# THUDM/GCC

Hardware: NVIDIA B200
Metric: subgraphs/sec (MoCo pretrain step) (higher is better)
Workload: dtype f32

## Files before the change

gcc_b200/csrc/gin_bwd.cu:

```cuda
#include "gin_common.cuh"
#include "tc_gemm.cuh"
#ifndef GCCB_EMU
#include <cuda_bf16.h>
#endif

namespace gccb {

#define GCCB_WG_CHUNKS 148

struct BwdLayout {
  size_t dh, g1[2], dz2[2], da, red, dS, dpool, part, total;
  size_t dz16, tA, tB, coef1, splitk;
  int DW;
  int cap_pad, splits;
};

inline BwdLayout make_bwd_layout(const GinDims& d, int B, int node_cap) {
  BwdLayout b;
  size_t off = 0;
  auto take = [&](size_t bytes) { size_t o = off; off += (bytes + 255) & ~(size_t)255; return o; };
  b.DW = d.H > GCCB_DINP ? d.H : GCCB_DINP;
  b.dh = take((size_t)node_cap * b.DW * 4);
  for (int i = 0; i < 2; ++i) {
    b.g1[i] = take((size_t)node_cap * d.H * 4);
    b.dz2[i] = take((size_t)node_cap * d.H * 4);
  }
  b.da = take((size_t)node_cap * b.DW * 4);
  b.red = take((size_t)(d.L - 1) * 3 * 2 * d.H * 8);
  b.dS = take((size_t)d.L * B * d.H * 4);
  b.dpool = take((size_t)d.L * B * b.DW * 4);
  b.part = take((size_t)GCCB_WG_CHUNKS * ((size_t)d.H * b.DW + d.H) * 4);
  b.dz16 = b.tA = b.tB = b.coef1 = b.splitk = 0;
  b.cap_pad = (node_cap + 63) & ~63;
  b.splits = 0;
#ifndef GCCB_EMU
  if (d.tc) {
    b.dz16 = take((size_t)node_cap * d.H * 2);
    b.tA = take((size_t)d.H * b.cap_pad * 2);
    b.tB = take((size_t)b.DW * b.cap_pad * 2);
    b.coef1 = take((size_t)(d.L - 1) * 2 * d.H * 4);
    const int tiles = (d.H / 128) * 1;
    b.splits = 148 / tiles;
    if (b.splits > b.cap_pad / 64) b.splits = b.cap_pad / 64;
// ... 90 lines not shown
  const int idx = blockIdx.x * blockDim.x + threadIdx.x;
  if (idx < H * inf) {
    const int o = idx / inf, k = idx - o * inf;
    float s = 0.f;
    for (int g = 0; g < B; ++g)
      s = fmaf(dS[((size_t)l * B + g) * H + o], pooled[((size_t)l * B + g) * PW + k], s);
    grads[lay.wp[l] + idx] += s;
  } else if (idx < H * inf + H) {
    const int o = idx - H * inf;
    float s = 0.f;
    for (int g = 0; g < B; ++g) s += dS[((size_t)l * B + g) * H + o];
    grads[lay.bp[l] + o] += s;
  }
}

template <int W>
__global__ void __launch_bounds__(256)
gin_bwd_dh_kernel(const int32_t* __restrict__ node_off_v, int B, const int32_t* __restrict__ indptr,
                  const int32_t* __restrict__ indices, const int32_t* __restrict__ graph_id,
                  const float* __restrict__ dpool_j, int DW, const float* __restrict__ da, int has_da,
                  float* __restrict__ dh) {
  __shared__ float scratch[8 * W];
  __shared__ int hub_rows[GCCB_HUB_QUEUE];
  __shared__ int n_hub;
  const int N = node_off_v[B];
  const int tid = threadIdx.x, lane = tid & 31, warp = tid >> 5;
  constexpr int V4 = W / 4, PERV = (V4 + 31) / 32;
  if (tid == 0) n_hub = 0;
  __syncthreads();
  for (int r = blockIdx.x * 8 + warp; r < N; r += gridDim.x * 8) {
    const int beg = indptr[r], end = indptr[r + 1];
    if (has_da && end - beg > GCCB_HUB_DEG) {
      int slot = GCCB_HUB_QUEUE;
      if (lane == 0) slot = atomicAdd(&n_hub, 1);
      slot = __shfl_sync(0xffffffffu, slot, 0);
      if (slot < GCCB_HUB_QUEUE) {
        if (lane == 0) hub_rows[slot] = r;
        continue;
      }
    }
    const int g = graph_id[r];
    float4 acc[PERV];
// ... 1 lines not shown
    for (int j = 0; j < PERV; ++j) {
      const int v = lane + 32 * j;
      acc[j] = make_float4(0.f, 0.f, 0.f, 0.f);
      if (v < V4) {
        acc[j] = *reinterpret_cast<const float4*>(dpool_j + (size_t)g * DW + 4 * v);
        if (has_da) {
          const float4 x = *reinterpret_cast<const float4*>(da + (size_t)r * W + 4 * v);
          acc[j].x += x.x; acc[j].y += x.y; acc[j].z += x.z; acc[j].w += x.w;
        }
      }
    }
    if (has_da) gather_range4<W>(da, indices, beg, end, lane, acc);
#pragma unroll
    for (int j = 0; j < PERV; ++j) {
      const int v = lane + 32 * j;
      if (v < V4) *reinterpret_cast<float4*>(dh + (size_t)r * W + 4 * v) = acc[j];
    }
  }
  __syncthreads();
  const int nh = min(n_hub, GCCB_HUB_QUEUE);
  for (int hi = 0; hi < nh; ++hi) {
    const int rh = hub_rows[hi];
    const float s = gather_hub<W>(da, indices, indptr[rh], indptr[rh + 1], scratch);
    if (tid < W) dh[(size_t)rh * W + tid] = dpool_j[(size_t)graph_id[rh] * DW + tid] + da[(size_t)rh * W + tid] + s;
  }
}

struct BnC { const float *mean, *invstd, *sc, *sh; };
__device__ __forceinline__ BnC bnc(const float* p, int H) { BnC b; b.mean = p; b.invstd = p + H; b.sc = p + 2 * H; b.sh = p + 3 * H; return b; }

__device__ __forceinline__ void chain_g4(float z2v, float dhv, const BnC& A, const BnC& Bc, int c,
                                         float* ya, float* yhat, float* g4) {
  float yap = fmaf(z2v, A.sc[c], A.sh[c]);
  float y = fmaxf(yap, 0.f);
  float hb = fmaf(y, Bc.sc[c], Bc.sh[c]);
  *ya = yap;
  *yhat = (y - Bc.mean[c]) * Bc.invstd[c];
  *g4 = hb > 0.f ? dhv : 0.f;
}

template <int H>
__global__ void __launch_bounds__(256)
gin_bwd_reduce_kernel(int mode, const int32_t* __restrict__ node_off_v, int B,
                      const float* __restrict__ z2, const float* __restrict__ dh,
                      const double* __restrict__ sums_a, const float* __restrict__ ga,
                      const float* __restrict__ bea, const double* __restrict__ sums_b,
                      const float* __restrict__ gb, const float* __restrict__ beb, float bn_eps,
                      const double* __restrict__ redB_in, double* __restrict__ red_out) {
  __shared__ float coef_a[4 * H];
  __shared__ float coef_b[4 * H];
  __shared__ float red[2 * 1024];
  const int N = node_off_v[B];
  const int tid = threadIdx.x;
  bn_prepare(sums_a, N, H, ga, bea, bn_eps, coef_a, coef_a + H, coef_a + 2 * H, coef_a + 3 * H, nullptr, false, false, 0.f);
  bn_prepare(sums_b, N, H, gb, beb, bn_eps, coef_b, coef_b + H, coef_b + 2 * H, coef_b + 3 * H, nullptr, false, false, 0.f);
  __syncthreads();
  const BnC A = bnc(coef_a, H), Bc = bnc(coef_b, H);
  constexpr int TPR = H / 4, RP = 256 / TPR;
  const int c4 = (tid % TPR) * 4, rsub = tid / TPR;
  const float invN = N > 0 ? 1.0f / (float)N : 0.f;
  float m_g4[4] = {0.f, 0.f, 0.f, 0.f}, m_g4y[4] = {0.f, 0.f, 0.f, 0.f};
  if (mode == 1) {
#pragma unroll
    for (int k = 0; k < 4; ++k) { m_g4[k] = (float)(redB_in[c4 + k] * invN); m_g4y[k] = (float)(redB_in[H + c4 + k] * invN); }
  }
  float s[4] = {0.f, 0.f, 0.f, 0.f}, q[4] = {0.f, 0.f, 0.f, 0.f};
  const int stride = gridDim.x * RP;
  for (int r = blockIdx.x * RP + rsub; r < N; r += 2 * stride) {
    float4 zv[2], dv[2];
#pragma unroll
    for (int u = 0; u < 2; ++u) {
      const int rr = r + u * stride;
      const bool ok = rr < N;
      zv[u] = ok ? *reinterpret_cast<const float4*>(z2 + (size_t)rr * H + c4) : make_float4(0.f, 0.f, 0.f, 0.f);
      dv[u] = ok ? *reinterpret_cast<const float4*>(dh + (size_t)rr * H + c4) : make_float4(0.f, 0.f, 0.f, 0.f);
    }
#pragma unroll
    for (int u = 0; u < 2; ++u) {
      if (r + u * stride < N) {
        const float zz[4] = {zv[u].x, zv[u].y, zv[u].z, zv[u].w}, dd[4] = {dv[u].x, dv[u].y, dv[u].z, dv[u].w};
#pragma unroll
        for (int k = 0; k < 4; ++k) {
          const int c = c4 + k;
          float ya, yhat, g4;
          chain_g4(zz[k], dd[k], A, Bc, c, &ya, &yhat, &g4);
          if (mode == 0) {
            s[k] += g4;
            q[k] = fmaf(g4, yhat, q[k]);
          } else {
            const float dy = Bc.sc[c] * (g4 - m_g4[k] - yhat * m_g4y[k]);
            const float g3 = ya > 0.f ? dy : 0.f;
            const float z2hat = (zz[k] - A.mean[c]) * A.invstd[c];
            s[k] += g3;
            q[k] = fmaf(g3, z2hat, q[k]);
          }
        }
      }
    }
  }
#pragma unroll
  for (int k = 0; k < 4; ++k) {
    red[(0 * RP + rsub) * H + c4 + k] = s[k];
    red[(RP + rsub) * H + c4 + k] = q[k];
  }
  __syncthreads();
  for (int idx = tid; idx < 2 * H; idx += 256) {
    int which = idx / H, cc = idx - which * H;
    float t = 0.f;
    for (int j = 0; j < RP; ++j) t += red[(which * RP + j) * H + cc];
    atomicAdd(&red_out[which * H + cc], (double)t);
// ... 151 lines not shown
#pragma unroll
    for (int i = 0; i < 4; ++i) {
      const int r = row0 + ty * 4 + i;
      if (r < N) {
#pragma unroll
        for (int c = 0; c < TC::CPT; ++c) da_out[(size_t)r * KIN + TC::col(tx, c)] = acc[i][c];
      }
    }
  }
}

__global__ void __launch_bounds__(256)
gin_wgrad_kernel(const int32_t* __restrict__ node_off_v, int B, int H, int KQ,
                 const float* __restrict__ P, const float* __restrict__ Q,
                 const double* __restrict__ q_sums, const float* __restrict__ q_gamma,
                 const float* __restrict__ q_beta, float bn_eps, float* __restrict__ part) {
  __shared__ float Ps[GCCB_TILE_ROWS][65];
  __shared__ float Qs[GCCB_TILE_ROWS][65];
  __shared__ float qsc[64], qsh[64];
  const int N = node_off_v[B];
  const int tid = threadIdx.x, tx = tid & 15, ty = tid >> 4;
  const int kblocks = (KQ + 63) / 64;
  const int ob = blockIdx.y / kblocks, kb = blockIdx.y - ob * kblocks;
  const int o0 = ob * 64, k0 = kb * 64;
  const bool xform = q_sums != nullptr;
  if (xform) {
    for (int c = tid; c < 64; c += 256) {
      int k = k0 + c;
      float sc = 0.f, sh = 0.f;
      if (k < KQ) {
        double n = N > 0 ? (double)N : 1.0;
// ... 48 lines not shown
    }
    if (kb == 0 && tid < 64)
      for (int rr = 0; rr < GCCB_TILE_ROWS; ++rr) bacc += Ps[rr][tid];
  }
  float* mypart = part + (size_t)blockIdx.x * ((size_t)H * KQ + H);
#pragma unroll
  for (int i = 0; i < 4; ++i) {
    int o = o0 + ty * 4 + i;
#pragma unroll
    for (int j = 0; j < 4; ++j) {
      int k = k0 + tx * 4 + j;
      if (o < H && k < KQ) mypart[(size_t)o * KQ + k] = acc[i][j];
    }
  }
  if (kb == 0 && tid < 64 && o0 + tid < H) mypart[(size_t)H * KQ + o0 + tid] = bacc;
}

__global__ void __launch_bounds__(256)
gin_wgrad_reduce_kernel(int H, int KQ, int in_features, const float* __restrict__ part,
                        float* __restrict__ gw, float* __restrict__ gb) {
  const int idx = blockIdx.x * blockDim.x + threadIdx.x;
  const size_t stride = (size_t)H * KQ + H;
  if (idx < H * KQ) {
    const int o = idx / KQ, k = idx - o * KQ;
    if (k < in_features) {
      float s0 = 0.f, s1 = 0.f, s2 = 0.f, s3 = 0.f;
      for (int ch = 0; ch < GCCB_WG_CHUNKS; ch += 4) {
        s0 += part[(ch + 0) * stride + idx]; s1 += part[(ch + 1) * stride + idx];
        s2 += part[(ch + 2) * stride + idx]; s3 += part[(ch + 3) * stride + idx];
      }
      gw[(size_t)o * in_features + k] += (s0 + s1) + (s2 + s3);
    }
  } else if (idx < H * KQ + H) {
    float s = 0.f;
    for (int ch = 0; ch < GCCB_WG_CHUNKS; ++ch) s += part[ch * stride + idx];
    gb[idx - H * KQ] += s;
  }
}

__global__ void gin_bn_grads_kernel(int H, const double* __restrict__ red, float* __restrict__ gw,
                                    float* __restrict__ gb) {
  int c = blockIdx.x * blockDim.x + threadIdx.x;
  if (c < H) { gb[c] += (float)red[c]; gw[c] += (float)red[H + c]; }
}

__global__ void __launch_bounds__(256)
gin_bwd_emb_kernel(GinDims d, const int32_t* __restrict__ node_off_v, int B,
                   const int32_t* __restrict__ sub_deg, const float* __restrict__ dx0,
                   float* __restrict__ gemb) {
  GCCB_DYN_SMEM(float, hist);
  const int N = node_off_v[B];
  const int cells = (d.maxdeg + 1) * d.D;
  for (int i = threadIdx.x; i < cells; i += blockDim.x) hist[i] = 0.f;
  __syncthreads();
  const int total = N * d.D;
  for (int idx = blockIdx.x * blockDim.x + threadIdx.x; idx < total; idx += gridDim.x * blockDim.x) {
    int r = idx / d.D, c = idx - r * d.D;
    int dg = sub_deg[r];
// ... 31 lines not shown
  const int32_t* node_off_v = a.batch->node_off + (size_t)a.view * (B + 1);
  const int32_t* indptr = a.batch->indptr + (size_t)a.view * (cap + 1);
  const int32_t* indices = a.batch->indices + (size_t)a.view * a.batch->edge_cap;
  const int32_t* sub_deg = a.batch->sub_deg + (size_t)a.view * cap;
  const int32_t* graph_id = a.batch->graph_id + (size_t)a.view * cap;
  const double* stats = (const double*)(a.acts + a.al.stats);
  float* dh = (float*)(a.ws + a.bl.dh);
  float* da = (float*)(a.ws + a.bl.da);
  double* red = (double*)(a.ws + a.bl.red);
  float* dS = (float*)(a.ws + a.bl.dS);
  float* dpool = (float*)(a.ws + a.bl.dpool);
  float* part = (float*)(a.ws + a.bl.part);
  const float* P = a.params;
  float* G = a.grads;
  const int DW = a.bl.DW;
  const int tiles = (cap + GCCB_TILE_ROWS - 1) / GCCB_TILE_ROWS;
  const int grid = tiles < 592 ? tiles : 592;
  const uint32_t keep = (uint32_t)fmin((1.0 - (double)d.drop_p) * 4294967296.0, 4294967295.0);
#ifndef GCCB_EMU
  StreamKit* kit = stream_kit((cudaStream_t)a.stream, 1);
  cudaStream_t main_s = (cudaStream_t)a.stream;
  gccb_stream_t side = kit->side[0];
  cudaEvent_t* ev_main = kit->ev;
  cudaEvent_t* ev_side = kit->ev + 8;
  cudaEvent_t ev_head = kit->ev[16], ev_join = kit->ev[17];
#else
  gccb_stream_t side = a.stream;
#endif
  cudaMemsetAsync(red, 0, (size_t)(d.L - 1) * 3 * 2 * H * sizeof(double), (cudaStream_t)a.stream);
  auto kpb = gin_pool_predict_bwd_kernel<H>;
  GCCB_LAUNCH(kpb, (B + GCCB_GPB - 1) / GCCB_GPB, 256, 0, a.stream, d, node_off_v, B, P, a.lay, (const float*)(a.acts + a.al.score),
              a.dfeat, a.drop_key, a.drop_step, a.drop_base, keep, DW, dS, dpool);
#ifndef GCCB_EMU
  cudaEventRecord(ev_head, main_s);
  cudaStreamWaitEvent((cudaStream_t)side, ev_head, 0);
#endif
  {
    int maxout = H * (d.din > H ? d.din : H) + H;
    dim3 gr((maxout + 255) / 256, d.L);
    GCCB_LAUNCH(gin_pred_wgrad_kernel, gr, 256, 0, side, d, B, a.lay, (const float*)dS,
                (const float*)(a.acts + a.al.pooled), a.al.PW, G);
  }
  for (int l = d.L - 2; l >= 0; --l) {
    float* g1 = (float*)(a.ws + a.bl.g1[l & 1]);
    float* dz2 = (float*)(a.ws + a.bl.dz2[l & 1]);
    const int j = l + 1;
    const float* z1 = (const float*)(a.acts + a.al.z1[l]);
    const float* z2 = (const float*)(a.acts + a.al.z2[l]);
    const float* a_l = (const float*)(a.acts + a.al.a[l]);
    const double* s1 = stats + (size_t)(l * 3 + 0) * 2 * H;
    const double* sa = stats + (size_t)(l * 3 + 1) * 2 * H;
    const double* sb = stats + (size_t)(l * 3 + 2) * 2 * H;
    double* r1 = red + (size_t)(l * 3 + 0) * 2 * H;
    double* rA = red + (size_t)(l * 3 + 1) * 2 * H;
    double* rB = red + (size_t)(l * 3 + 2) * 2 * H;
    auto kdh = gin_bwd_dh_kernel<H>;
    GCCB_LAUNCH(kdh, (tiles < 1184 ? tiles : 1184), 256, 0, a.stream, node_off_v, B, indptr, indices, graph_id,
                (const float*)(dpool + (size_t)j * B * DW), DW, (const float*)da, j < d.L - 1 ? 1 : 0, dh);
    auto kred = gin_bwd_reduce_kernel<H>;
    GCCB_LAUNCH(kred, grid, 256, 0, a.stream, 0, node_off_v, B, z2, (const float*)dh, sa, P + a.lay.bna_w[l],
                P + a.lay.bna_b[l], sb, P + a.lay.bnb_w[l], P + a.lay.bnb_b[l], d.bn_eps,
                (const double*)rB, rB);
    GCCB_LAUNCH(kred, grid, 256, 0, a.stream, 1, node_off_v, B, z2, (const float*)dh, sa, P + a.lay.bna_w[l],
                P + a.lay.bna_b[l], sb, P + a.lay.bnb_w[l], P + a.lay.bnb_b[l], d.bn_eps,
                (const double*)rB, rA);
#ifndef GCCB_EMU
    if (l + 2 <= d.L - 2) cudaStreamWaitEvent(main_s, ev_side[l + 2], 0);
#endif
    {
      auto k = gin_bwd_gemm2_kernel<H>;
      size_t sm = ((size_t)GCCB_TILE_ROWS * (H + 1) + (size_t)GCCB_KC * (H + 4) + 2 * 16 * H + 16 * H) * 4;
      gccb::ensure_dyn_smem(k, sm);
      GCCB_LAUNCH(k, grid, 256, sm, a.stream, node_off_v, B, z1, z2, (const float*)dh, s1, P + a.lay.bn1_w[l],
                  P + a.lay.bn1_b[l], sa, P + a.lay.bna_w[l], P + a.lay.bna_b[l], sb, P + a.lay.bnb_w[l],
                  P + a.lay.bnb_b[l], d.bn_eps, (const double*)rB, (const double*)rA, P + a.lay.w2[l], dz2,
                  g1, r1);
    }
    const int KQ1 = gin_in_width(d, l), inf = gin_in_features(d, l);
// ... 3 lines not shown
      gccb::ensure_dyn_smem(k, sm);
      GCCB_LAUNCH(k, grid, 256, sm, a.stream, node_off_v, B, z1, g1, s1, P + a.lay.bn1_w[l], P + a.lay.bn1_b[l],
                  d.bn_eps, (const double*)r1, P + a.lay.w1[l], inf, da);
    } else {
      auto k = gin_bwd_gemm1_kernel<H, H>;
      size_t sm = ((size_t)GCCB_TILE_ROWS * (H + 1) + (size_t)GCCB_KC * (H + 4) + 6 * H) * 4;
      gccb::ensure_dyn_smem(k, sm);
      GCCB_LAUNCH(k, grid, 256, sm, a.stream, node_off_v, B, z1, g1, s1, P + a.lay.bn1_w[l], P + a.lay.bn1_b[l],
                  d.bn_eps, (const double*)r1, P + a.lay.w1[l], inf, da);
    }
#ifndef GCCB_EMU
    cudaEventRecord(ev_main[l], main_s);
    cudaStreamWaitEvent((cudaStream_t)side, ev_main[l], 0);
#endif
    {
      dim3 gr(GCCB_WG_CHUNKS, ((H + 63) / 64) * ((H + 63) / 64));
      GCCB_LAUNCH(gin_wgrad_kernel, gr, 256, 0, side, node_off_v, B, H, H, (const float*)dz2, z1, s1,
                  P + a.lay.bn1_w[l], P + a.lay.bn1_b[l], d.bn_eps, part);
      GCCB_LAUNCH(gin_wgrad_reduce_kernel, (H * H + H + 255) / 256, 256, 0, side, H, H, H,
                  (const float*)part, G + a.lay.w2[l], G + a.lay.b2[l]);
      dim3 gr1(GCCB_WG_CHUNKS, ((H + 63) / 64) * ((KQ1 + 63) / 64));
      GCCB_LAUNCH(gin_wgrad_kernel, gr1, 256, 0, side, node_off_v, B, H, KQ1, (const float*)g1, a_l,
                  (const double*)nullptr, (const float*)nullptr, (const float*)nullptr, d.bn_eps, part);
      GCCB_LAUNCH(gin_wgrad_reduce_kernel, (H * KQ1 + H + 255) / 256, 256, 0, side, H, KQ1, inf,
                  (const float*)part, G + a.lay.w1[l], G + a.lay.b1[l]);
    }
    GCCB_LAUNCH(gin_bn_grads_kernel, (H + 127) / 128, 128, 0, side, H, (const double*)rB,
                G + a.lay.bnb_w[l], G + a.lay.bnb_b[l]);
    GCCB_LAUNCH(gin_bn_grads_kernel, (H + 127) / 128, 128, 0, side, H, (const double*)rA,
                G + a.lay.bna_w[l], G + a.lay.bna_b[l]);
    GCCB_LAUNCH(gin_bn_grads_kernel, (H + 127) / 128, 128, 0, side, H, (const double*)r1,
                G + a.lay.bn1_w[l], G + a.lay.bn1_b[l]);
#ifndef GCCB_EMU
    cudaEventRecord(ev_side[l], (cudaStream_t)side);
#endif
  }
  auto kdh0 = gin_bwd_dh_kernel<GCCB_DINP>;
  GCCB_LAUNCH(kdh0, (tiles < 1184 ? tiles : 1184), 256, 0, a.stream, node_off_v, B, indptr, indices, graph_id, (const float*)dpool, DW,
              (const float*)da, 1, dh);
  {
    size_t sm = (size_t)(d.maxdeg + 1) * d.D * sizeof(float);
    auto k = gin_bwd_emb_kernel;
    gccb::ensure_dyn_smem(k, sm);
    GCCB_LAUNCH(k, 64, 256, sm, a.stream, d, node_off_v, B, sub_deg, (const float*)dh, G + a.lay.emb);
  }
#ifndef GCCB_EMU
  cudaEventRecord(ev_join, (cudaStream_t)side);
  cudaStreamWaitEvent(main_s, ev_join, 0);
#endif
  return check_launch("gccb_gin_backward");
}


#ifndef GCCB_EMU
// ... 195 lines not shown
  __nv_bfloat16* tB = (__nv_bfloat16*)(a.ws + a.bl.tB);
  float* coef1 = (float*)(a.ws + a.bl.coef1);
  float* splitk = (float*)(a.ws + a.bl.splitk);
  const float* P = a.params;
  float* G = a.grads;
  const int DW = a.bl.DW, capP = a.bl.cap_pad;
  const int tiles = (cap + GCCB_TILE_ROWS - 1) / GCCB_TILE_ROWS;
  const int grid = tiles < 592 ? tiles : 592;
  const uint32_t keep = (uint32_t)fmin((1.0 - (double)d.drop_p) * 4294967296.0, 4294967295.0);
  StreamKit* kit = stream_kit((cudaStream_t)a.stream, 1);
  cudaStream_t main_s = (cudaStream_t)a.stream;
  cudaStream_t side = kit->side[0];
  cudaEvent_t* ev_main = kit->ev;
  cudaEvent_t* ev_side = kit->ev + 8;
  cudaEvent_t ev_head = kit->ev[16], ev_join = kit->ev[17];
  cudaMemsetAsync(red, 0, (size_t)(d.L - 1) * 3 * 2 * H * sizeof(double), main_s);
  auto kpb = gin_pool_predict_bwd_kernel<H>;
  GCCB_LAUNCH(kpb, (B + GCCB_GPB - 1) / GCCB_GPB, 256, 0, a.stream, d, node_off_v, B, P, a.lay, (const float*)(a.acts + a.al.score),
              a.dfeat, a.drop_key, a.drop_step, a.drop_base, keep, DW, dS, dpool);
  cudaEventRecord(ev_head, main_s);
  cudaStreamWaitEvent(side, ev_head, 0);
  {
    int maxout = H * (d.din > H ? d.din : H) + H;
    dim3 gr((maxout + 255) / 256, d.L);
    GCCB_LAUNCH(gin_pred_wgrad_kernel, gr, 256, 0, side, d, B, a.lay, (const float*)dS,
                (const float*)(a.acts + a.al.pooled), a.al.PW, G);
  }
  for (int l = d.L - 2; l >= 0; --l) {
    float* g1 = (float*)(a.ws + a.bl.g1[l & 1]);
    float* dz2 = (float*)(a.ws + a.bl.dz2[l & 1]);
    const int j = l + 1;
    const float* z1 = (const float*)(a.acts + a.al.z1[l]);
    const float* z2 = (const float*)(a.acts + a.al.z2[l]);
    const float* a_l = (const float*)(a.acts + a.al.a[l]);
    const double* s1 = stats + (size_t)(l * 3 + 0) * 2 * H;
    const double* sa = stats + (size_t)(l * 3 + 1) * 2 * H;
    const double* sb = stats + (size_t)(l * 3 + 2) * 2 * H;
    double* r1 = red + (size_t)(l * 3 + 0) * 2 * H;
    double* rA = red + (size_t)(l * 3 + 1) * 2 * H;
    double* rB = red + (size_t)(l * 3 + 2) * 2 * H;
    const int KW = gin_kw(d, l), inf = gin_in_features(d, l);
    const __nv_bfloat16* w1b = (const __nv_bfloat16*)(a.acts + a.al.w16[l]);
    const __nv_bfloat16* w1t = w1b + (size_t)H * KW + (size_t)H * H;
    const __nv_bfloat16* w2t = w1t + (size_t)KW * H;
    float* c1 = coef1 + (size_t)l * 2 * H;
    auto kdh = gin_bwd_dh_kernel<H>;
    GCCB_LAUNCH(kdh, (tiles < 1184 ? tiles : 1184), 256, 0, a.stream, node_off_v, B, indptr, indices, graph_id,
                (const float*)(dpool + (size_t)j * B * DW), DW, (const float*)da, j < d.L - 1 ? 1 : 0, dh);
    auto kred = gin_bwd_reduce_kernel<H>;
    GCCB_LAUNCH(kred, grid, 256, 0, a.stream, 0, node_off_v, B, z2, (const float*)dh, sa, P + a.lay.bna_w[l],
                P + a.lay.bna_b[l], sb, P + a.lay.bnb_w[l], P + a.lay.bnb_b[l], d.bn_eps, (const double*)rB, rB);
    GCCB_LAUNCH(kred, grid, 256, 0, a.stream, 1, node_off_v, B, z2, (const float*)dh, sa, P + a.lay.bna_w[l],
                P + a.lay.bna_b[l], sb, P + a.lay.bnb_w[l], P + a.lay.bnb_b[l], d.bn_eps, (const double*)rB, rA);
    if (l + 2 <= d.L - 2) cudaStreamWaitEvent(main_s, ev_side[l + 2], 0);
    auto kz2 = gin_bwd_dz2_kernel<H>;
    GCCB_LAUNCH(kz2, grid, 256, 0, a.stream, node_off_v, B, z2, (const float*)dh, s1, P + a.lay.bn1_w[l],
                P + a.lay.bn1_b[l], sa, P + a.lay.bna_w[l], P + a.lay.bna_b[l], sb, P + a.lay.bnb_w[l],
                P + a.lay.bnb_b[l], d.bn_eps, (const double*)rB, (const double*)rA, dz2, dz16, c1);
    int rc = tc::gemm_bf16(dz16, w2t, cap, H, H, n_dev, nullptr, 1.0f, g1, nullptr, H, nullptr, 1, nullptr, main_s);
    if (rc) return rc;
    auto kg1 = gin_bwd_g1_kernel<H>;
    GCCB_LAUNCH(kg1, grid, 256, 0, a.stream, node_off_v, B, z1, g1, s1, P + a.lay.bn1_w[l], P + a.lay.bn1_b[l],
                d.bn_eps, r1);
    auto kz1 = gin_bwd_dz1_kernel<H>;
    GCCB_LAUNCH(kz1, grid, 256, 0, a.stream, node_off_v, B, z1, g1, s1, P + a.lay.bn1_w[l], P + a.lay.bn1_b[l],
                d.bn_eps, (const double*)r1, dz16);
    rc = tc::gemm_bf16(dz16, w1t, cap, KW, H, n_dev, nullptr, 1.0f, da, nullptr, KW, nullptr, 1, nullptr, main_s);
    if (rc) return rc;
    cudaEventRecord(ev_main[l], main_s);
    cudaStreamWaitEvent(side, ev_main[l], 0);
    rc = tc::cast_bf16(dz2, cap, H, H, tA, capP, H, 1, n_dev, side);
    if (!rc) rc = tc::cast_bf16(z1, cap, H, H, tB, capP, H, 1, n_dev, side, c1, c1 + H, 1);
    if (!rc) rc = tc::gemm_bf16(tA, tB, H, H, capP, nullptr, nullptr, 1.0f, G + a.lay.w2[l], nullptr, H, nullptr,
                                a.bl.splits, splitk, side, 1.0f, H);
    if (!rc) rc = tc::cast_bf16(g1, cap, H, H, tA, capP, H, 1, n_dev, side);
    if (!rc) rc = tc::cast_bf16(a_l, cap, KW, KW, tB, capP, KW, 1, n_dev, side);
    if (!rc) rc = tc::gemm_bf16(tA, tB, H, KW, capP, nullptr, nullptr, 1.0f, G + a.lay.w1[l], nullptr, inf, nullptr,
                                a.bl.splits, splitk, side, 1.0f, inf);
    if (rc) return rc;
    GCCB_LAUNCH(gin_bn_grads_kernel, (H + 127) / 128, 128, 0, side, H, (const double*)rB,
                G + a.lay.bnb_w[l], G + a.lay.bnb_b[l]);
    GCCB_LAUNCH(gin_bn_grads_kernel, (H + 127) / 128, 128, 0, side, H, (const double*)rA,
                G + a.lay.bna_w[l], G + a.lay.bna_b[l]);
    GCCB_LAUNCH(gin_bn_grads_kernel, (H + 127) / 128, 128, 0, side, H, (const double*)r1,
                G + a.lay.bn1_w[l], G + a.lay.bn1_b[l]);
    cudaEventRecord(ev_side[l], side);
  }
  auto kdh0 = gin_bwd_dh_kernel<GCCB_DINP>;
  GCCB_LAUNCH(kdh0, (tiles < 1184 ? tiles : 1184), 256, 0, a.stream, node_off_v, B, indptr, indices, graph_id, (const float*)dpool, DW,
              (const float*)da, 1, dh);
  {
    size_t sm = (size_t)(d.maxdeg + 1) * d.D * sizeof(float);
    auto k = gin_bwd_emb_kernel;
    gccb::ensure_dyn_smem(k, sm);
    GCCB_LAUNCH(k, 64, 256, sm, a.stream, d, node_off_v, B, sub_deg, (const float*)dh, G + a.lay.emb);
  }
  cudaEventRecord(ev_join, side);
  cudaStreamWaitEvent(main_s, ev_join, 0);
  return check_launch("gccb_gin_backward (tensor cores)");
}
#endif

}

using namespace gccb;
// ... 40 lines not shown
```

gcc_b200/csrc/gin_common.cuh:

```cuda
#pragma once
#include "common.cuh"

namespace gccb {

#define GCCB_DINP 64
#define GCCB_TILE_ROWS 64
#define GCCB_KC 64
#define GCCB_MAX_L 8

struct GinDims {
  int L, H, P, D, maxdeg, din;
  int norm;
  int tc;
  float bn_eps, bn_mom, norm_eps, drop_p;
};

__host__ __device__ __forceinline__ int gin_in_features(const GinDims& d, int l) { return l == 0 ? d.din : d.H; }
__host__ __device__ __forceinline__ int gin_in_width(const GinDims& d, int l) { return l == 0 ? GCCB_DINP : d.H; }

struct ActsLayout {
  size_t x0;
  size_t a[GCCB_MAX_L], z1[GCCB_MAX_L], z2[GCCB_MAX_L], h[GCCB_MAX_L];
  size_t stats;
  size_t pool_acc;
// ... 292 lines not shown
```

gcc_b200/csrc/gin_fwd.cu:

```cuda
#include "gin_common.cuh"
#include "tc_gemm.cuh"
#ifndef GCCB_EMU
#include <cuda_bf16.h>
#endif

namespace gccb {

__global__ void __launch_bounds__(256)
gin_build_x0_kernel(GinDims d, const int32_t* __restrict__ node_off_v, int B,
                    const float* __restrict__ pos, const int32_t* __restrict__ sub_deg,
                    const int32_t* __restrict__ graph_id, const float* __restrict__ emb,
                    float* __restrict__ x0) {
  const int N = node_off_v[B];
  const int total = N * GCCB_DINP;
  for (int idx = blockIdx.x * blockDim.x + threadIdx.x; idx < total; idx += gridDim.x * blockDim.x) {
    int r = idx / GCCB_DINP, c = idx - r * GCCB_DINP;
    float v = 0.f;
    if (c < d.P) {
      v = pos[(size_t)r * d.P + c];
    } else if (c < d.P + d.D) {
      int dg = sub_deg[r];
      dg = dg < 0 ? 0 : (dg > d.maxdeg ? d.maxdeg : dg);
      v = emb[(size_t)dg * d.D + (c - d.P)];
    } else if (c == d.P + d.D) {
// ... 416 lines not shown
};

template <int H>
static int run_forward(const FwdArgs& a) {
  const GinDims& d = a.d;
  const int B = a.batch->batch, cap = a.batch->node_cap;
  const int32_t* node_off_v = a.batch->node_off + (size_t)a.view * (B + 1);
  const int32_t* indptr = a.batch->indptr + (size_t)a.view * (cap + 1);
  const int32_t* indices = a.batch->indices + (size_t)a.view * a.batch->edge_cap;
  const int32_t* sub_deg = a.batch->sub_deg + (size_t)a.view * cap;
  const int32_t* graph_id = a.batch->graph_id + (size_t)a.view * cap;
  const float* pos_v = a.pos + (size_t)a.view * cap * d.P;
  float* x0 = (float*)(a.acts + a.al.x0);
  double* stats = (double*)(a.acts + a.al.stats);
  const int tiles = (cap + GCCB_TILE_ROWS - 1) / GCCB_TILE_ROWS;
  const int grid = tiles < 592 ? tiles : 592;
  const int use_running = a.bn_train ? 0 : 1, upd = a.bn_train ? 1 : 0;
  cudaMemsetAsync(stats, 0, a.al.pool_acc + (size_t)d.L * B * a.al.PW * sizeof(double) - a.al.stats,
                  (cudaStream_t)a.stream);
  GCCB_LAUNCH(gin_build_x0_kernel, grid, 256, 0, a.stream, d, node_off_v, B, pos_v, sub_deg, graph_id,
              a.params + a.lay.emb, x0);
  const float* hin = x0;
  for (int l = 0; l < d.L - 1; ++l) {
    float* a_l = (float*)(a.acts + a.al.a[l]);
    float* z1 = (float*)(a.acts + a.al.z1[l]);
    float* z2 = (float*)(a.acts + a.al.z2[l]);
    float* hout = (float*)(a.acts + a.al.h[l]);
    double* s1 = stats + (size_t)(l * 3 + 0) * 2 * H;
    double* sa = stats + (size_t)(l * 3 + 1) * 2 * H;
    double* sb = stats + (size_t)(l * 3 + 2) * 2 * H;
    float* run1 = a.running ? a.running + (size_t)(l * 3 + 0) * 2 * H : nullptr;
// ... 314 lines not shown
```

Before: 264,200.

## Fuse BN reductions into dh kernel and wgrad reduce into wgrad tail

Folds the first BN backward reduction (mode 0) into the dh gather kernel, which removes one full pass over z2/dh per layer. The weight-gradient partial reduction now runs inside gin_wgrad_kernel using last-block-done tickets in two hierarchical stages, which removes a separate reduce launch. The per-layer BN grad launches are merged into a single kernel at the end. The costs are more shared memory and register pressure in the dh kernel, double atomics, and serialized tail blocks in wgrad.

```diff
diff --git a/gcc_b200/csrc/gin_bwd.cu b/gcc_b200/csrc/gin_bwd.cu
--- a/gcc_b200/csrc/gin_bwd.cu
+++ b/gcc_b200/csrc/gin_bwd.cu
@@ -7,6 +7,17 @@
 namespace gccb {
 
 #define GCCB_WG_CHUNKS 148
+#define GCCB_WG_GROUP 16
+#define GCCB_WG_NG ((GCCB_WG_CHUNKS + GCCB_WG_GROUP - 1) / GCCB_WG_GROUP)
+#define GCCB_WG_CNT 256
+
+#ifdef GCCB_EMU
+__device__ __forceinline__ float4 ld_cg4(const float* p) { return *reinterpret_cast<const float4*>(p); }
+__device__ __forceinline__ float ld_cg(const float* p) { return *p; }
+#else
+__device__ __forceinline__ float4 ld_cg4(const float* p) { return __ldcg(reinterpret_cast<const float4*>(p)); }
+__device__ __forceinline__ float ld_cg(const float* p) { return __ldcg(p); }
+#endif
 
 struct BwdLayout {
   size_t dh, g1[2], dz2[2], da, red, dS, dpool, part, total;
@@ -14,6 +25,10 @@
   int DW;
   int cap_pad, splits;
 };
+
+inline size_t bwd_red_bytes(const GinDims& d) {
+  return (size_t)(d.L - 1) * 3 * 2 * d.H * 8 + (size_t)(d.L - 1) * 2 * GCCB_WG_CNT * 4;
+}
 
 inline BwdLayout make_bwd_layout(const GinDims& d, int B, int node_cap) {
   BwdLayout b;
@@ -26,7 +41,7 @@
     b.dz2[i] = take((size_t)node_cap * d.H * 4);
   }
   b.da = take((size_t)node_cap * b.DW * 4);
-  b.red = take((size_t)(d.L - 1) * 3 * 2 * d.H * 8);
+  b.red = take(bwd_red_bytes(d));
   b.dS = take((size_t)d.L * B * d.H * 4);
   b.dpool = take((size_t)d.L * B * b.DW * 4);
   b.part = take((size_t)GCCB_WG_CHUNKS * ((size_t)d.H * b.DW + d.H) * 4);
@@ -147,18 +162,53 @@
   }
 }
 
-template <int W>
+struct BnC { const float *mean, *invstd, *sc, *sh; };
+__device__ __forceinline__ BnC bnc(const float* p, int H) { BnC b; b.mean = p; b.invstd = p + H; b.sc = p + 2 * H; b.sh = p + 3 * H; return b; }
+
+__device__ __forceinline__ void chain_g4(float z2v, float dhv, const BnC& A, const BnC& Bc, int c,
+                                         float* ya, float* yhat, float* g4) {
+  float yap = fmaf(z2v, A.sc[c], A.sh[c]);
+  float y = fmaxf(yap, 0.f);
+  float hb = fmaf(y, Bc.sc[c], Bc.sh[c]);
+  *ya = yap;
+  *yhat = (y - Bc.mean[c]) * Bc.invstd[c];
+  *g4 = hb > 0.f ? dhv : 0.f;
+}
+
+struct DhBn {
+  const float* z2;
+  const double *sums_a, *sums_b;
+  const float *ga, *bea, *gb, *beb;
+  float eps;
+  double* red_out;
+};
+
+template <int W, bool BN>
 __global__ void __launch_bounds__(256)
 gin_bwd_dh_kernel(const int32_t* __restrict__ node_off_v, int B, const int32_t* __restrict__ indptr,
                   const int32_t* __restrict__ indices, const int32_t* __restrict__ graph_id,
                   const float* __restrict__ dpool_j, int DW, const float* __restrict__ da, int has_da,
-                  float* __restrict__ dh) {
-  __shared__ float scratch[8 * W];
+                  float* __restrict__ dh, DhBn bn) {
+  __shared__ float scratch[BN ? 18 * W : 8 * W];
   __shared__ int hub_rows[GCCB_HUB_QUEUE];
   __shared__ int n_hub;
+  __shared__ float coef[BN ? 8 * W : 1];
+  float* red = scratch;
   const int N = node_off_v[B];
   const int tid = threadIdx.x, lane = tid & 31, warp = tid >> 5;
   constexpr int V4 = W / 4, PERV = (V4 + 31) / 32;
+  if (BN) {
+    bn_prepare(bn.sums_a, N, W, bn.ga, bn.bea, bn.eps, coef, coef + W, coef + 2 * W, coef + 3 * W, nullptr, false,
+               false, 0.f);
+    bn_prepare(bn.sums_b, N, W, bn.gb, bn.beb, bn.eps, coef + 4 * W, coef + 5 * W, coef + 6 * W, coef + 7 * W, nullptr,
+               false, false, 0.f);
+  }
+  const BnC A = bnc(coef, W), Bc = bnc(coef + 4 * W, W);
+  float s[PERV][4], q[PERV][4];
+#pragma unroll
+  for (int j = 0; j < PERV; ++j)
+#pragma unroll
+    for (int k = 0; k < 4; ++k) s[j][k] = q[j][k] = 0.f;
   if (tid == 0) n_hub = 0;
   __syncthreads();
   for (int r = blockIdx.x * 8 + warp; r < N; r += gridDim.x * 8) {
@@ -190,34 +240,65 @@
 #pragma unroll
     for (int j = 0; j < PERV; ++j) {
       const int v = lane + 32 * j;
-      if (v < V4) *reinterpret_cast<float4*>(dh + (size_t)r * W + 4 * v) = acc[j];
-    }
-  }
-  __syncthreads();
+      if (v < V4) {
+        *reinterpret_cast<float4*>(dh + (size_t)r * W + 4 * v) = acc[j];
+        if (BN) {
+          const float4 z = *reinterpret_cast<const float4*>(bn.z2 + (size_t)r * W + 4 * v);
+          const float zz[4] = {z.x, z.y, z.z, z.w}, dd[4] = {acc[j].x, acc[j].y, acc[j].z, acc[j].w};
+#pragma unroll
+          for (int k = 0; k < 4; ++k) {
+            float ya, yhat, g4;
+            chain_g4(zz[k], dd[k], A, Bc, 4 * v + k, &ya, &yhat, &g4);
+            s[j][k] += g4;
+            q[j][k] = fmaf(g4, yhat, q[j][k]);
+          }
+        }
+      }
+    }
+  }
+  __syncthreads();
+  float hs = 0.f, hq = 0.f;
   const int nh = min(n_hub, GCCB_HUB_QUEUE);
   for (int hi = 0; hi < nh; ++hi) {
     const int rh = hub_rows[hi];
-    const float s = gather_hub<W>(da, indices, indptr[rh], indptr[rh + 1], scratch);
-    if (tid < W) dh[(size_t)rh * W + tid] = dpool_j[(size_t)graph_id[rh] * DW + tid] + da[(size_t)rh * W + tid] + s;
-  }
-}
-
-struct BnC { const float *mean, *invstd, *sc, *sh; };
-__device__ __forceinline__ BnC bnc(const float* p, int H) { BnC b; b.mean = p; b.invstd = p + H; b.sc = p + 2 * H; b.sh = p + 3 * H; return b; }
-
-__device__ __forceinline__ void chain_g4(float z2v, float dhv, const BnC& A, const BnC& Bc, int c,
-                                         float* ya, float* yhat, float* g4) {
-  float yap = fmaf(z2v, A.sc[c], A.sh[c]);
-  float y = fmaxf(yap, 0.f);
-  float hb = fmaf(y, Bc.sc[c], Bc.sh[c]);
-  *ya = yap;
-  *yhat = (y - Bc.mean[c]) * Bc.invstd[c];
-  *g4 = hb > 0.f ? dhv : 0.f;
+    const float sn = gather_hub<W>(da, indices, indptr[rh], indptr[rh + 1], scratch);
+    if (tid < W) {
+      const float v = dpool_j[(size_t)graph_id[rh] * DW + tid] + da[(size_t)rh * W + tid] + sn;
+      dh[(size_t)rh * W + tid] = v;
+      if (BN) {
+        float ya, yhat, g4;
+        chain_g4(bn.z2[(size_t)rh * W + tid], v, A, Bc, tid, &ya, &yhat, &g4);
+        hs += g4;
+        hq = fmaf(g4, yhat, hq);
+      }
+    }
+  }
+  if constexpr (BN) {
+#pragma unroll
+    for (int j = 0; j < PERV; ++j) {
+      const int v = lane + 32 * j;
+      if (v < V4)
+#pragma unroll
+        for (int k = 0; k < 4; ++k) {
+          red[(0 * 8 + warp) * W + 4 * v + k] = s[j][k];
+          red[(1 * 8 + warp) * W + 4 * v + k] = q[j][k];
+        }
+    }
+    if (tid < W) { red[16 * W + tid] = hs; red[17 * W + tid] = hq; }
+    __syncthreads();
+    for (int idx = tid; idx < 2 * W; idx += 256) {
+      const int which = idx / W, c = idx - which * W;
+      float t = red[16 * W + idx];
+#pragma unroll
+      for (int w = 0; w < 8; ++w) t += red[(which * 8 + w) * W + c];
+      atomicAdd(&bn.red_out[idx], (double)t);
+    }
+  }
 }
 
 template <int H>
-__global__ void __launch_bounds__(256)
-gin_bwd_reduce_kernel(int mode, const int32_t* __restrict__ node_off_v, int B,
+__global__ void __launch_bounds__(256, H <= 64 ? 4 : 1)
+gin_bwd_reduce_kernel(const int32_t* __restrict__ node_off_v, int B,
                       const float* __restrict__ z2, const float* __restrict__ dh,
                       const double* __restrict__ sums_a, const float* __restrict__ ga,
                       const float* __restrict__ bea, const double* __restrict__ sums_b,
@@ -235,11 +316,9 @@
   constexpr int TPR = H / 4, RP = 256 / TPR;
   const int c4 = (tid % TPR) * 4, rsub = tid / TPR;
   const float invN = N > 0 ? 1.0f / (float)N : 0.f;
-  float m_g4[4] = {0.f, 0.f, 0.f, 0.f}, m_g4y[4] = {0.f, 0.f, 0.f, 0.f};
-  if (mode == 1) {
-#pragma unroll
-    for (int k = 0; k < 4; ++k) { m_g4[k] = (float)(redB_in[c4 + k] * invN); m_g4y[k] = (float)(redB_in[H + c4 + k] * invN); }
-  }
+  float m_g4[4], m_g4y[4];
+#pragma unroll
+  for (int k = 0; k < 4; ++k) { m_g4[k] = (float)(redB_in[c4 + k] * invN); m_g4y[k] = (float)(redB_in[H + c4 + k] * invN); }
   float s[4] = {0.f, 0.f, 0.f, 0.f}, q[4] = {0.f, 0.f, 0.f, 0.f};
   const int stride = gridDim.x * RP;
   for (int r = blockIdx.x * RP + rsub; r < N; r += 2 * stride) {
@@ -260,16 +339,11 @@
           const int c = c4 + k;
           float ya, yhat, g4;
           chain_g4(zz[k], dd[k], A, Bc, c, &ya, &yhat, &g4);
-          if (mode == 0) {
-            s[k] += g4;
-            q[k] = fmaf(g4, yhat, q[k]);
-          } else {
-            const float dy = Bc.sc[c] * (g4 - m_g4[k] - yhat * m_g4y[k]);
-            const float g3 = ya > 0.f ? dy : 0.f;
-            const float z2hat = (zz[k] - A.mean[c]) * A.invstd[c];
-            s[k] += g3;
-            q[k] = fmaf(g3, z2hat, q[k]);
-          }
+          const float dy = Bc.sc[c] * (g4 - m_g4[k] - yhat * m_g4y[k]);
+          const float g3 = ya > 0.f ? dy : 0.f;
+          const float z2hat = (zz[k] - A.mean[c]) * A.invstd[c];
+          s[k] += g3;
+          q[k] = fmaf(g3, z2hat, q[k]);
         }
       }
     }
@@ -451,7 +525,8 @@
 gin_wgrad_kernel(const int32_t* __restrict__ node_off_v, int B, int H, int KQ,
                  const float* __restrict__ P, const float* __restrict__ Q,
                  const double* __restrict__ q_sums, const float* __restrict__ q_gamma,
-                 const float* __restrict__ q_beta, float bn_eps, float* __restrict__ part) {
+                 const float* __restrict__ q_beta, float bn_eps, float* __restrict__ part,
+                 unsigned* __restrict__ cnt, int in_features, float* __restrict__ gw, float* __restrict__ gb) {
   __shared__ float Ps[GCCB_TILE_ROWS][65];
   __shared__ float Qs[GCCB_TILE_ROWS][65];
   __shared__ float qsc[64], qsh[64];
@@ -530,34 +605,75 @@
     }
   }
   if (kb == 0 && tid < 64 && o0 + tid < H) mypart[(size_t)H * KQ + o0 + tid] = bacc;
-}
-
-__global__ void __launch_bounds__(256)
-gin_wgrad_reduce_kernel(int H, int KQ, int in_features, const float* __restrict__ part,
-                        float* __restrict__ gw, float* __restrict__ gb) {
-  const int idx = blockIdx.x * blockDim.x + threadIdx.x;
+  __shared__ unsigned ticket;
   const size_t stride = (size_t)H * KQ + H;
-  if (idx < H * KQ) {
-    const int o = idx / KQ, k = idx - o * KQ;
-    if (k < in_features) {
-      float s0 = 0.f, s1 = 0.f, s2 = 0.f, s3 = 0.f;
-      for (int ch = 0; ch < GCCB_WG_CHUNKS; ch += 4) {
-        s0 += part[(ch + 0) * stride + idx]; s1 += part[(ch + 1) * stride + idx];
-        s2 += part[(ch + 2) * stride + idx]; s3 += part[(ch + 3) * stride + idx];
-      }
-      gw[(size_t)o * in_features + k] += (s0 + s1) + (s2 + s3);
-    }
-  } else if (idx < H * KQ + H) {
-    float s = 0.f;
-    for (int ch = 0; ch < GCCB_WG_CHUNKS; ++ch) s += part[ch * stride + idx];
-    gb[idx - H * KQ] += s;
-  }
-}
-
-__global__ void gin_bn_grads_kernel(int H, const double* __restrict__ red, float* __restrict__ gw,
-                                    float* __restrict__ gb) {
-  int c = blockIdx.x * blockDim.x + threadIdx.x;
-  if (c < H) { gb[c] += (float)red[c]; gw[c] += (float)red[H + c]; }
+  const int grp = blockIdx.x / GCCB_WG_GROUP, c_beg = grp * GCCB_WG_GROUP;
+  const int c_n = min(GCCB_WG_GROUP, GCCB_WG_CHUNKS - c_beg);
+  unsigned* my_cnt = cnt + (size_t)blockIdx.y * (GCCB_WG_NG + 1);
+  const int ro = o0 + (tid >> 2), rk = k0 + (tid & 3) * 16;
+  auto sum_slots = [&](int first, int n, int step, float4 (&w)[4], float& bsum) {
+#pragma unroll
+    for (int i = 0; i < 4; ++i) w[i] = make_float4(0.f, 0.f, 0.f, 0.f);
+    bsum = 0.f;
+#pragma unroll 4
+    for (int t = 0; t < n; ++t) {
+      const float* src = part + (size_t)(first + t * step) * stride;
+      if (ro < H) {
+#pragma unroll
+        for (int i = 0; i < 4; ++i)
+          if (rk + 4 * i < KQ) {
+            const float4 x = ld_cg4(src + (size_t)ro * KQ + rk + 4 * i);
+            w[i].x += x.x; w[i].y += x.y; w[i].z += x.z; w[i].w += x.w;
+          }
+      }
+      if (kb == 0 && tid < 64 && o0 + tid < H) bsum += ld_cg(src + (size_t)H * KQ + o0 + tid);
+    }
+  };
+  __threadfence();
+  __syncthreads();
+  if (tid == 0) ticket = atomicAdd(&my_cnt[grp], 1u);
+  __syncthreads();
+  if (ticket != (unsigned)c_n - 1) return;
+  __threadfence();
+  float4 w[4];
+  float bsum;
+  sum_slots(c_beg, c_n, 1, w, bsum);
+  float* slot = part + (size_t)c_beg * stride;
+  if (ro < H)
+#pragma unroll
+    for (int i = 0; i < 4; ++i)
+      if (rk + 4 * i < KQ) *reinterpret_cast<float4*>(slot + (size_t)ro * KQ + rk + 4 * i) = w[i];
+  if (kb == 0 && tid < 64 && o0 + tid < H) slot[(size_t)H * KQ + o0 + tid] = bsum;
+  __threadfence();
+  __syncthreads();
+  if (tid == 0) ticket = atomicAdd(&my_cnt[GCCB_WG_NG], 1u);
+  __syncthreads();
+  if (ticket != (unsigned)GCCB_WG_NG - 1) return;
+  __threadfence();
+  sum_slots(0, GCCB_WG_NG, GCCB_WG_GROUP, w, bsum);
+  if (ro < H)
+#pragma unroll
+    for (int i = 0; i < 4; ++i) {
+      const float v[4] = {w[i].x, w[i].y, w[i].z, w[i].w};
+#pragma unroll
+      for (int e = 0; e < 4; ++e) {
+        const int k = rk + 4 * i + e;
+        if (k < in_features) gw[(size_t)ro * in_features + k] += v[e];
+      }
+    }
+  if (kb == 0 && tid < 64 && o0 + tid < H) gb[o0 + tid] += bsum;
+}
+
+__global__ void gin_bn_grads_kernel(int L, int H, gccb_gin_layout_t lay, const double* __restrict__ red,
+                                    float* __restrict__ G) {
+  const int i = blockIdx.x * blockDim.x + threadIdx.x;
+  if (i >= (L - 1) * 3 * H) return;
+  const int c = i % H, lb = i / H, l = lb / 3, which = lb - 3 * l;
+  const double* r = red + (size_t)lb * 2 * H;
+  const int64_t w = which == 0 ? lay.bn1_w[l] : which == 1 ? lay.bna_w[l] : lay.bnb_w[l];
+  const int64_t b = which == 0 ? lay.bn1_b[l] : which == 1 ? lay.bna_b[l] : lay.bnb_b[l];
+  G[b + c] += (float)r[c];
+  G[w + c] += (float)r[H + c];
 }
 
 __global__ void __launch_bounds__(256)
@@ -619,8 +735,10 @@
   const float* P = a.params;
   float* G = a.grads;
   const int DW = a.bl.DW;
+  unsigned* wg_cnt = (unsigned*)(red + (size_t)(d.L - 1) * 3 * 2 * H);
   const int tiles = (cap + GCCB_TILE_ROWS - 1) / GCCB_TILE_ROWS;
-  const int grid = tiles < 592 ? tiles : 592;
+  const int grid = tiles < GCCB_GIN_GRID ? tiles : GCCB_GIN_GRID;
+  const int row_grid = tiles < GCCB_GIN_ROW_GRID ? tiles : GCCB_GIN_ROW_GRID;
   const uint32_t keep = (uint32_t)fmin((1.0 - (double)d.drop_p) * 4294967296.0, 4294967295.0);
 #ifndef GCCB_EMU
   StreamKit* kit = stream_kit((cudaStream_t)a.stream, 1);
@@ -632,7 +750,7 @@
 #else
   gccb_stream_t side = a.stream;
 #endif
-  cudaMemsetAsync(red, 0, (size_t)(d.L - 1) * 3 * 2 * H * sizeof(double), (cudaStream_t)a.stream);
+  cudaMemsetAsync(red, 0, bwd_red_bytes(d), (cudaStream_t)a.stream);
   auto kpb = gin_pool_predict_bwd_kernel<H>;
   GCCB_LAUNCH(kpb, (B + GCCB_GPB - 1) / GCCB_GPB, 256, 0, a.stream, d, node_off_v, B, P, a.lay, (const float*)(a.acts + a.al.score),
               a.dfeat, a.drop_key, a.drop_step, a.drop_base, keep, DW, dS, dpool);
@@ -659,14 +777,13 @@
     double* r1 = red + (size_t)(l * 3 + 0) * 2 * H;
     double* rA = red + (size_t)(l * 3 + 1) * 2 * H;
     double* rB = red + (size_t)(l * 3 + 2) * 2 * H;
-    auto kdh = gin_bwd_dh_kernel<H>;
-    GCCB_LAUNCH(kdh, (tiles < 1184 ? tiles : 1184), 256, 0, a.stream, node_off_v, B, indptr, indices, graph_id,
-                (const float*)(dpool + (size_t)j * B * DW), DW, (const float*)da, j < d.L - 1 ? 1 : 0, dh);
+    const DhBn bn = {z2, sa, sb, P + a.lay.bna_w[l], P + a.lay.bna_b[l], P + a.lay.bnb_w[l], P + a.lay.bnb_b[l],
+                     d.bn_eps, rB};
+    auto kdh = gin_bwd_dh_kernel<H, true>;
+    GCCB_LAUNCH(kdh, row_grid, 256, 0, a.stream, node_off_v, B, indptr, indices, graph_id,
+                (const float*)(dpool + (size_t)j * B * DW), DW, (const float*)da, j < d.L - 1 ? 1 : 0, dh, bn);
     auto kred = gin_bwd_reduce_kernel<H>;
-    GCCB_LAUNCH(kred, grid, 256, 0, a.stream, 0, node_off_v, B, z2, (const float*)dh, sa, P + a.lay.bna_w[l],
-                P + a.lay.bna_b[l], sb, P + a.lay.bnb_w[l], P + a.lay.bnb_b[l], d.bn_eps,
-                (const double*)rB, rB);
-    GCCB_LAUNCH(kred, grid, 256, 0, a.stream, 1, node_off_v, B, z2, (const float*)dh, sa, P + a.lay.bna_w[l],
+    GCCB_LAUNCH(kred, grid, 256, 0, a.stream, node_off_v, B, z2, (const float*)dh, sa, P + a.lay.bna_w[l],
                 P + a.lay.bna_b[l], sb, P + a.lay.bnb_w[l], P + a.lay.bnb_b[l], d.bn_eps,
                 (const double*)rB, rA);
 #ifndef GCCB_EMU
@@ -700,30 +817,24 @@
     cudaStreamWaitEvent((cudaStream_t)side, ev_main[l], 0);
 #endif
     {
+      unsigned* cnt = wg_cnt + (size_t)l * 2 * GCCB_WG_CNT;
       dim3 gr(GCCB_WG_CHUNKS, ((H + 63) / 64) * ((H + 63) / 64));
       GCCB_LAUNCH(gin_wgrad_kernel, gr, 256, 0, side, node_off_v, B, H, H, (const float*)dz2, z1, s1,
-                  P + a.lay.bn1_w[l], P + a.lay.bn1_b[l], d.bn_eps, part);
-      GCCB_LAUNCH(gin_wgrad_reduce_kernel, (H * H + H + 255) / 256, 256, 0, side, H, H, H,
-                  (const float*)part, G + a.lay.w2[l], G + a.lay.b2[l]);
+                  P + a.lay.bn1_w[l], P + a.lay.bn1_b[l], d.bn_eps, part, cnt, H, G + a.lay.w2[l], G + a.lay.b2[l]);
       dim3 gr1(GCCB_WG_CHUNKS, ((H + 63) / 64) * ((KQ1 + 63) / 64));
       GCCB_LAUNCH(gin_wgrad_kernel, gr1, 256, 0, side, node_off_v, B, H, KQ1, (const float*)g1, a_l,
-                  (const double*)nullptr, (const float*)nullptr, (const float*)nullptr, d.bn_eps, part);
-      GCCB_LAUNCH(gin_wgrad_reduce_kernel, (H * KQ1 + H + 255) / 256, 256, 0, side, H, KQ1, inf,
-                  (const float*)part, G + a.lay.w1[l], G + a.lay.b1[l]);
-    }
-    GCCB_LAUNCH(gin_bn_grads_kernel, (H + 127) / 128, 128, 0, side, H, (const double*)rB,
-                G + a.lay.bnb_w[l], G + a.lay.bnb_b[l]);
-    GCCB_LAUNCH(gin_bn_grads_kernel, (H + 127) / 128, 128, 0, side, H, (const double*)rA,
-                G + a.lay.bna_w[l], G + a.lay.bna_b[l]);
-    GCCB_LAUNCH(gin_bn_grads_kernel, (H + 127) / 128, 128, 0, side, H, (const double*)r1,
-                G + a.lay.bn1_w[l], G + a.lay.bn1_b[l]);
+                  (const double*)nullptr, (const float*)nullptr, (const float*)nullptr, d.bn_eps, part,
+                  cnt + GCCB_WG_CNT, inf, G + a.lay.w1[l], G + a.lay.b1[l]);
+    }
 #ifndef GCCB_EMU
     cudaEventRecord(ev_side[l], (cudaStream_t)side);
 #endif
   }
-  auto kdh0 = gin_bwd_dh_kernel<GCCB_DINP>;
-  GCCB_LAUNCH(kdh0, (tiles < 1184 ? tiles : 1184), 256, 0, a.stream, node_off_v, B, indptr, indices, graph_id, (const float*)dpool, DW,
-              (const float*)da, 1, dh);
+  GCCB_LAUNCH(gin_bn_grads_kernel, ((d.L - 1) * 3 * H + 255) / 256, 256, 0, side, d.L, H, a.lay,
+              (const double*)red, G);
+  auto kdh0 = gin_bwd_dh_kernel<GCCB_DINP, false>;
+  GCCB_LAUNCH(kdh0, row_grid, 256, 0, a.stream, node_off_v, B, indptr, indices, graph_id, (const float*)dpool, DW,
+              (const float*)da, 1, dh, DhBn{});
   {
     size_t sm = (size_t)(d.maxdeg + 1) * d.D * sizeof(float);
     auto k = gin_bwd_emb_kernel;
@@ -949,7 +1060,7 @@
   cudaEvent_t* ev_main = kit->ev;
   cudaEvent_t* ev_side = kit->ev + 8;
   cudaEvent_t ev_head = kit->ev[16], ev_join = kit->ev[17];
-  cudaMemsetAsync(red, 0, (size_t)(d.L - 1) * 3 * 2 * H * sizeof(double), main_s);
+  cudaMemsetAsync(red, 0, bwd_red_bytes(d), main_s);
   auto kpb = gin_pool_predict_bwd_kernel<H>;
   GCCB_LAUNCH(kpb, (B + GCCB_GPB - 1) / GCCB_GPB, 256, 0, a.stream, d, node_off_v, B, P, a.lay, (const float*)(a.acts + a.al.score),
               a.dfeat, a.drop_key, a.drop_step, a.drop_base, keep, DW, dS, dpool);
@@ -979,13 +1090,13 @@
     const __nv_bfloat16* w1t = w1b + (size_t)H * KW + (size_t)H * H;
     const __nv_bfloat16* w2t = w1t + (size_t)KW * H;
     float* c1 = coef1 + (size_t)l * 2 * H;
-    auto kdh = gin_bwd_dh_kernel<H>;
+    const DhBn bn = {z2, sa, sb, P + a.lay.bna_w[l], P + a.lay.bna_b[l], P + a.lay.bnb_w[l], P + a.lay.bnb_b[l],
+                     d.bn_eps, rB};
+    auto kdh = gin_bwd_dh_kernel<H, true>;
     GCCB_LAUNCH(kdh, (tiles < 1184 ? tiles : 1184), 256, 0, a.stream, node_off_v, B, indptr, indices, graph_id,
-                (const float*)(dpool + (size_t)j * B * DW), DW, (const float*)da, j < d.L - 1 ? 1 : 0, dh);
+                (const float*)(dpool + (size_t)j * B * DW), DW, (const float*)da, j < d.L - 1 ? 1 : 0, dh, bn);
     auto kred = gin_bwd_reduce_kernel<H>;
-    GCCB_LAUNCH(kred, grid, 256, 0, a.stream, 0, node_off_v, B, z2, (const float*)dh, sa, P + a.lay.bna_w[l],
-                P + a.lay.bna_b[l], sb, P + a.lay.bnb_w[l], P + a.lay.bnb_b[l], d.bn_eps, (const double*)rB, rB);
-    GCCB_LAUNCH(kred, grid, 256, 0, a.stream, 1, node_off_v, B, z2, (const float*)dh, sa, P + a.lay.bna_w[l],
+    GCCB_LAUNCH(kred, grid, 256, 0, a.stream, node_off_v, B, z2, (const float*)dh, sa, P + a.lay.bna_w[l],
                 P + a.lay.bna_b[l], sb, P + a.lay.bnb_w[l], P + a.lay.bnb_b[l], d.bn_eps, (const double*)rB, rA);
     if (l + 2 <= d.L - 2) cudaStreamWaitEvent(main_s, ev_side[l + 2], 0);
     auto kz2 = gin_bwd_dz2_kernel<H>;
@@ -1013,17 +1124,13 @@
     if (!rc) rc = tc::gemm_bf16(tA, tB, H, KW, capP, nullptr, nullptr, 1.0f, G + a.lay.w1[l], nullptr, inf, nullptr,
                                 a.bl.splits, splitk, side, 1.0f, inf);
     if (rc) return rc;
-    GCCB_LAUNCH(gin_bn_grads_kernel, (H + 127) / 128, 128, 0, side, H, (const double*)rB,
-                G + a.lay.bnb_w[l], G + a.lay.bnb_b[l]);
-    GCCB_LAUNCH(gin_bn_grads_kernel, (H + 127) / 128, 128, 0, side, H, (const double*)rA,
-                G + a.lay.bna_w[l], G + a.lay.bna_b[l]);
-    GCCB_LAUNCH(gin_bn_grads_kernel, (H + 127) / 128, 128, 0, side, H, (const double*)r1,
-                G + a.lay.bn1_w[l], G + a.lay.bn1_b[l]);
     cudaEventRecord(ev_side[l], side);
   }
-  auto kdh0 = gin_bwd_dh_kernel<GCCB_DINP>;
+  GCCB_LAUNCH(gin_bn_grads_kernel, ((d.L - 1) * 3 * H + 255) / 256, 256, 0, side, d.L, H, a.lay,
+              (const double*)red, G);
+  auto kdh0 = gin_bwd_dh_kernel<GCCB_DINP, false>;
   GCCB_LAUNCH(kdh0, (tiles < 1184 ? tiles : 1184), 256, 0, a.stream, node_off_v, B, indptr, indices, graph_id, (const float*)dpool, DW,
-              (const float*)da, 1, dh);
+              (const float*)da, 1, dh, DhBn{});
   {
     size_t sm = (size_t)(d.maxdeg + 1) * d.D * sizeof(float);
     auto k = gin_bwd_emb_kernel;
diff --git a/gcc_b200/csrc/gin_common.cuh b/gcc_b200/csrc/gin_common.cuh
--- a/gcc_b200/csrc/gin_common.cuh
+++ b/gcc_b200/csrc/gin_common.cuh
@@ -7,6 +7,13 @@
 #define GCCB_TILE_ROWS 64
 #define GCCB_KC 64
 #define GCCB_MAX_L 8
+
+#ifndef GCCB_GIN_GRID
+#define GCCB_GIN_GRID 592
+#endif
+#ifndef GCCB_GIN_ROW_GRID
+#define GCCB_GIN_ROW_GRID 1184
+#endif
 
 struct GinDims {
   int L, H, P, D, maxdeg, din;
diff --git a/gcc_b200/csrc/gin_fwd.cu b/gcc_b200/csrc/gin_fwd.cu
--- a/gcc_b200/csrc/gin_fwd.cu
+++ b/gcc_b200/csrc/gin_fwd.cu
@@ -454,7 +454,7 @@
   float* x0 = (float*)(a.acts + a.al.x0);
   double* stats = (double*)(a.acts + a.al.stats);
   const int tiles = (cap + GCCB_TILE_ROWS - 1) / GCCB_TILE_ROWS;
-  const int grid = tiles < 592 ? tiles : 592;
+  const int grid = tiles < GCCB_GIN_GRID ? tiles : GCCB_GIN_GRID;
   const int use_running = a.bn_train ? 0 : 1, upd = a.bn_train ? 1 : 0;
   cudaMemsetAsync(stats, 0, a.al.pool_acc + (size_t)d.L * B * a.al.PW * sizeof(double) - a.al.stats,
                   (cudaStream_t)a.stream);
diff --git a/profiles/compare_dumps.py b/profiles/compare_dumps.py
--- /dev/null
+++ b/profiles/compare_dumps.py
@@ -0,0 +1,25 @@
+#!/usr/bin/env python
+import os
+import sys
+
+import numpy as np
+
+a_dir, b_dir = sys.argv[1], sys.argv[2]
+exact = sys.argv[sys.argv.index("--exact") + 1].split(",") if "--exact" in sys.argv else []
+bad = 0
+for name in sorted(os.listdir(a_dir)):
+    a = np.load(os.path.join(a_dir, name))
+    b = np.load(os.path.join(b_dir, name))
+    key = name[:-4]
+    if a.shape != b.shape:
+        print("%-14s shape %s vs %s" % (key, a.shape, b.shape))
+        bad += 1
+        continue
+    d = float(np.max(np.abs(a.astype(np.float64) - b))) if a.size else 0.0
+    scale = float(np.max(np.abs(a))) if a.size else 0.0
+    same = np.array_equal(a, b)
+    print("%-14s max|diff| %.3e  rel %.3e  %s" % (key, d, d / scale if scale else 0.0, "identical" if same else ""))
+    if key in exact and not same:
+        print("  ^ must be identical")
+        bad += 1
+sys.exit(1 if bad else 0)
```

Result: slower. 260,600 (median of 6 runs) (-1.4%).
